# yesint/molar

Measured on AMD Instinct MI355X. Metric: frames/sec + Matom-pairs/sec, 1M-atom PBC neighbor search + RMSD fit, higher is better.
Workload: dtype f32; 1 GPU; 1M-atom synthetic triclinic box A, per frame: PBC neighbour search rc=1.2 nm (ordered pair list in HBM) + Kabsch RMSD fit/COM/gyration of a 100k-atom selection; natoms=1000000, selection_atoms=100000, frames_per_gpu=1451, parallelism=frames sharded over 1 rank(s), no data-path collective, streams_per_gpu=2, measure_overlapped_with_search=True

## Files before the change

molar_amd/csrc/pair_kernels.hpp:

```cpp
#pragma once

#include "boxmath.hpp"
#include "common.hpp"

namespace mh {
namespace pairk {

enum { MODE_COUNT = 0, MODE_FILL = 1, MODE_HIST = 2 };

#ifndef MH_COUNT_WPE
#define MH_COUNT_WPE 6
#endif
#ifndef MH_FILL_WPE
#define MH_FILL_WPE 8
#endif
#ifndef MH_WPB
#define MH_WPB 1
#endif
constexpr int waves_per_block(int mode) { return mode == MODE_HIST ? 4 : MH_WPB; }
constexpr int KREG = 8;
constexpr int FIFO_CAP = 128;
#ifndef MOLAR_HIP_NO_WIDE_FLUSH
#define MOLAR_HIP_WIDE_FLUSH 1
#endif
constexpr int FIFO_WIDE = 256;
constexpr uint32_t XCD_RUN = 128;
constexpr float F32_EPS = 1.1920929e-07f;
constexpr bool MASKED_COUNT_SORTED = true;

static __constant__ uint8_t MASKS[14][6] = {
    {0, 0, 0, 0, 0, 0},
    {0, 0, 0, 1, 0, 0}, {0, 0, 0, 0, 1, 0}, {0, 0, 0, 0, 0, 1},
    {0, 0, 0, 1, 1, 0}, {0, 0, 0, 1, 0, 1}, {0, 0, 0, 0, 1, 1},
    {0, 0, 0, 1, 1, 1},
    {1, 0, 0, 0, 1, 0}, {1, 0, 0, 0, 0, 1}, {0, 1, 0, 0, 0, 1},
    {1, 1, 0, 0, 0, 1}, {1, 0, 1, 0, 1, 0}, {0, 1, 1, 1, 0, 0},
};


typedef float v4f_t __attribute__((ext_vector_type(4)));
__device__ __forceinline__ float4 gload4(const float4 *p, size_t i) {
    const v4f_t v = ((const __attribute__((address_space(1))) v4f_t *)p)[i];
    return make_float4(v.x, v.y, v.z, v.w);
}
__device__ __forceinline__ uint32_t gload_u32(const uint32_t *p, size_t i) {
    return ((const __attribute__((address_space(1))) uint32_t *)p)[i];
}
__device__ __forceinline__ void gstore_u32(uint32_t *p, size_t i, uint32_t v) {
    ((__attribute__((address_space(1))) uint32_t *)p)[i] = v;
}
__device__ __forceinline__ float uniform_f32(float v) { return __uint_as_float(__builtin_amdgcn_readfirstlane(__float_as_uint(v))); }
__device__ __forceinline__ float4 lload4(const float4 *p, uint32_t i) {
    const v4f_t v = ((const __attribute__((address_space(3))) v4f_t *)p)[i];
    return make_float4(v.x, v.y, v.z, v.w);
}

struct SearchParams {
    const float4 *sa;
    const float4 *sb;
    const uint32_t *csa;
    const uint32_t *csb;
    const float *vdwa;
    const float *vdwb;
    const float4 *aabb_b;
    const float4 *perm_b;
    const float4 *chunk_aabb_b;
    const uint4 *h16_b;
    const float4 *cell_org_b;
    uint32_t mfma_count;
    const struct TaskDesc *task_desc;
    uint32_t *maskbuf;
    const unsigned long long *task_moff;
    unsigned long long mask_cap_units;
    unsigned long long out_cap;
    uint32_t dx, dy, dz;
    uint32_t pbc;
    uint32_t use_box;
    uint32_t nblocks;
    uint32_t wrap_kind;
    uint32_t prune_wrapped;
    float prune_limit2;
    uint32_t approx_wrapped;
    float band_lo, band_hi;
    uint32_t hist_nbins;
    float hist_min, hist_max;
    unsigned long long *hist_bins;
    unsigned long long *hist_total;
    const float *hist_edges;
    float hist_scale;
    uint32_t hist_lean;
    const uint32_t *hist_nslots;
#ifdef MOLAR_HIP_DEBUG_KNOBS
    uint32_t debug_skip;
    unsigned long long *dbg;
#endif
    float cutoff2;
    uint64_t ntasks;
    molar_hip_box box;
    alignas(16) float shifts4[96];
    uint32_t hist_big;
};

struct TaskDesc {
    uint32_t a0, n1, b0, n2, cb, flags, pad0, pad1;
};

struct SlotDesc {
    uint32_t a0, n1, b0, n2;
    uint32_t cb, flags, i0, frame;
    unsigned long long moff, pad1;
};
static_assert(sizeof(SlotDesc) == 48, "SlotDesc is read with three 16-byte loads");

struct Task {
    uint32_t a0, n1, b0, n2;
    uint32_t rps;
    uint32_t cb;
    uint32_t ca;
    uint32_t wrap_b;
    uint32_t wrap;
    bool tri;
    bool valid;
};

template <int KIND, bool UNIFORM>
__device__ __forceinline__ Task decode_task(const SearchParams &P, uint64_t t) {
    Task T;
    T.valid = false;
    T.tri = false;
    T.a0 = T.b0 = T.n1 = T.n2 = 0;
    T.cb = 0;
    T.ca = 0;
    T.wrap_b = 0;
    T.rps = 64u;
    T.wrap = 0;
    uint32_t half = 0;
    uint64_t e = t;
    if (KIND != MOLAR_HIP_SEARCH_SINGLE) {
        half = (uint32_t)(t & 1ull);
        e = t >> 1;
    }
    const uint32_t m = (uint32_t)(e % 14ull);
    const uint64_t cidx = e / 14ull;
    const uint32_t z = (uint32_t)(cidx % P.dz);
    const uint64_t r = cidx / P.dz;
    const uint32_t y = (uint32_t)(r % P.dy);
    const uint32_t x = (uint32_t)(r / P.dy);
    const uint32_t dims[3] = {P.dx, P.dy, P.dz};
    uint32_t c[2][3] = {{x + MASKS[m][0], y + MASKS[m][1], z + MASKS[m][2]},
                        {x + MASKS[m][3], y + MASKS[m][4], z + MASKS[m][5]}};
    uint32_t wrap = 0, wrap_c2 = 0;
    for (int i = 0; i < 2; ++i)
        for (int d = 0; d < 3; ++d)
            if (c[i][d] == dims[d]) {
                if ((P.pbc >> d) & 1u) {
                    c[i][d] = 0;
                    wrap |= 1u << d;
                    if (i == 1) wrap_c2 |= 1u << d;
                } else {
                    return T;
                }
            }
    const uint32_t i1 = c[0][0] + c[0][1] * P.dx + c[0][2] * P.dx * P.dy;
    const uint32_t i2 = c[1][0] + c[1][1] * P.dx + c[1][2] * P.dx * P.dy;
    uint32_t ca = i1, cb = i2;
    if (KIND == MOLAR_HIP_SEARCH_SINGLE) {
        T.tri = (i1 == i2);
    } else if (half) {
        ca = i2;
        cb = i1;
    }
    T.a0 = P.csa[ca];
    T.n1 = P.csa[ca + 1] - T.a0;
    T.b0 = P.csb[cb];
    T.n2 = P.csb[cb + 1] - T.b0;
    T.wrap = wrap;
    T.wrap_b = (KIND != MOLAR_HIP_SEARCH_SINGLE && half) ? (wrap & ~wrap_c2) : wrap_c2;
    T.rps = (P.use_box && wrap == MOLAR_HIP_PBC_FULL && P.box.nshift != 0 && T.n1 <= 4096u) ? (T.n1 <= 1024u ? 2u : 8u) : 64u;
    T.cb = cb;
    T.ca = ca;
    if (UNIFORM) {
        T.cb = __builtin_amdgcn_readfirstlane(T.cb);
        T.rps = __builtin_amdgcn_readfirstlane(T.rps);
        T.a0 = __builtin_amdgcn_readfirstlane(T.a0);
        T.n1 = __builtin_amdgcn_readfirstlane(T.n1);
        T.b0 = __builtin_amdgcn_readfirstlane(T.b0);
        T.n2 = __builtin_amdgcn_readfirstlane(T.n2);
        T.wrap = __builtin_amdgcn_readfirstlane(T.wrap);
    }
    T.valid = T.n1 > 0 && T.n2 > 0 && !(T.tri && T.n1 < 2);
    return T;
}

typedef float v2f __attribute__((ext_vector_type(2)));

enum { WK_NONE = 0, WK_DIAG = 1, WK_UPPER = 2, WK_GENERAL = 3 };

__device__ __forceinline__ v2f round_away2(v2f f) { return v2f{__builtin_roundf(f.x), __builtin_roundf(f.y)}; }

struct BoxRegs {
    float I[9], M[9];
    int nshift;
};

template <int WK, bool WIDE4 = false>
__device__ __forceinline__ v2f pair_d2x2(const SearchParams &P, const BoxRegs &B, uint32_t wrap, float px, float py,
                                         float pz, v2f qx, v2f qy, v2f qz) {
// ... 602 lines not shown
    typedef __attribute__((address_space(3))) uint32_t lds_u32;
    typedef __attribute__((address_space(1))) u4_t glb_u4;
    const float cutoff2 = P.cutoff2;
    const uint32_t rows = __builtin_amdgcn_readfirstlane(T.n1 - i0 < 64u ? T.n1 - i0 : 64u);
    const uint32_t kh = lane >> 5, cl = lane & 31u;
    const uint32_t nct = (T.n2 + 31u) >> 5, nch = (T.n2 + 63u) >> 6;
    float Sx = 0.f, Sy = 0.f, Sz = 0.f;
    for (int d = 0; d < 3; ++d) {
        if (!((T.wrap >> d) & 1u)) continue;
        const float sgn = ((T.wrap_b >> d) & 1u) ? 1.0f : -1.0f;
        Sx += sgn * P.box.m[3 * d];
        Sy += sgn * P.box.m[3 * d + 1];
        Sz += sgn * P.box.m[3 * d + 2];
    }
    float4 a = make_float4(0.f, 0.f, 0.f, 0.f);
    if (lane < rows) a = gload4(P.sa, T.a0 + i0 + lane);
    const float4 org = gload4(P.cell_org_b, T.cb);
    const float4 blo = gload4(P.aabb_b, 2 * T.cb), bhi = gload4(P.aabb_b, 2 * T.cb + 1);
    const bool need = lane < rows && !(aabb_d2(a.x - Sx, a.y - Sy, a.z - Sz, blo.x, blo.y, blo.z, bhi.x, bhi.y, bhi.z) > P.prune_limit2);
    const unsigned long long live = __builtin_amdgcn_ballot_w64(need);
    const uint32_t nlive = (uint32_t)__popcll(live);
    if (nlive == 0u) {
        count_out = 0u;
        return true;
    }
    const uint32_t rank = __builtin_amdgcn_mbcnt_hi((uint32_t)(live >> 32), __builtin_amdgcn_mbcnt_lo((uint32_t)live, 0u));
    const float r0 = (a.x - Sx) - org.x, r1 = (a.y - Sy) - org.y, r2 = (a.z - Sz) - org.z;
    float ra2 = need ? (r0 * r0 + r1 * r1) + r2 * r2 : 0.0f;
    float big = need ? fmaxf(fmaxf(fabsf(a.x), fabsf(a.y)), fabsf(a.z)) : 0.0f;
    const bool fin = ra2 == ra2;
    for (int off = 32; off > 0; off >>= 1) {
        ra2 = fmaxf(ra2, __shfl_xor(ra2, off, 64));
        big = fmaxf(big, __shfl_xor(big, off, 64));
    }
    const float R = 1.0001f * __builtin_sqrtf(ra2) + org.w;
    const float rc = __builtin_sqrtf(P.band_hi);
    const float L = (fmaxf(fmaxf(fabsf(org.x), fabsf(org.y)), fabsf(org.z)) + R) + (fmaxf(fmaxf(fabsf(Sx), fabsf(Sy)), fabsf(Sz)) + big);
    const float Em = mfma_error_bound(R, cutoff2);
    const float E = uniform_f32((P.band_hi - cutoff2) * 1.0001f + Em + 4.0f * (5.9604645e-08f * (2.0f * L + 2.0f * rc)) * rc);
    if (__builtin_amdgcn_ballot_w64(!fin || !(E == E) || !mfma_bound_usable(R, Em, cutoff2) || !(E < 0.06f * cutoff2)) != 0ull) return false;
    u4_t bq[MFMA_TILES];
#pragma unroll
    for (int t = 0; t < MFMA_TILES; ++t) {
        const uint32_t col = (uint32_t)t * 32u + cl;
        if (32u * (uint32_t)(t + 1) <= T.n2) {
            bq[t] = ((const glb_u4 *)P.h16_b)[T.b0 + col];
        } else {
            bq[t] = u4_t{0u, 0u, 0u, 0x00007BFFu};
            if (col < T.n2) bq[t] = ((const glb_u4 *)P.h16_b)[T.b0 + col];
        }
    }
    {
        ((lds_u4 *)lh)[2u * lane] = u4_t{0u, 0u, 0u, 0x00007BFFu};
        ((lds_u4 *)lh)[2u * lane + 1u] = u4_t{0u, 0u, 0u, 0x3C003C00u};
        __builtin_amdgcn_wave_barrier();
        if (need) {
            const _Float16 h0 = (_Float16)r0, h1 = (_Float16)r1, h2 = (_Float16)r2;
            const _Float16 l0 = (_Float16)(r0 - (float)h0), l1 = (_Float16)(r1 - (float)h1), l2 = (_Float16)(r2 - (float)h2);
            const float e0 = (float)h0 + (float)l0, e1 = (float)h1 + (float)l1, e2 = (float)h2 + (float)l2;
            const float na = ((e0 * e0 + e1 * e1) + e2 * e2) - cutoff2;
            const _Float16 nh = (_Float16)na, nl = (_Float16)(na - (float)nh);
            const _Float16 m2 = (_Float16)-2.0f;
            const _Float16 g0 = m2 * h0, g1 = m2 * h1, g2 = m2 * h2, s0 = m2 * l0, s1 = m2 * l1, s2 = m2 * l2;
            ((lds_u4 *)lh)[2u * rank] = u4_t{pack_h2(g0, g1), pack_h2(g2, g0), pack_h2(g1, g2), pack_h2(nh, nl)};
            ((lds_u4 *)lh)[2u * rank + 1u] = u4_t{pack_h2(s0, s1), pack_h2(s2, s0), pack_h2(s1, s2), 0x3C003C00u};
            la[rank] = a;
        }
    }
    __builtin_amdgcn_wave_barrier();
    const u4_t a0q = ((const lds_u4 *)lh)[2u * cl + kh], a1q = ((const lds_u4 *)lh)[2u * (32u + cl) + kh];
    const v8h_t A0 = __builtin_bit_cast(v8h_t, a0q), A1 = __builtin_bit_cast(v8h_t, a1q);
    __builtin_amdgcn_wave_barrier();
    lds_u32 *todo = (lds_u32 *)lh;
    constexpr uint32_t TODO_CAP = 512u;
    uint32_t ntodo = 0, cnt = 0;
    const uint32_t ngroups = nlive > 32u ? 2u : 1u;
    auto block = [&](int t, int rt) __attribute__((always_inline)) -> uint32_t {
        u4_t bt = bq[t];
        if (kh == 0u) bt.w = 0x3C003C00u;
        const v16f_t zero = {0.f, 0.f, 0.f, 0.f, 0.f, 0.f, 0.f, 0.f, 0.f, 0.f, 0.f, 0.f, 0.f, 0.f, 0.f, 0.f};
        const v16f_t acc = __builtin_amdgcn_mfma_f32_32x32x16_f16(rt == 0 ? A0 : A1, __builtin_bit_cast(v8h_t, bt), zero, 0, 0, 0);
        uint32_t h = 0u;
        float m = INFINITY;
#pragma unroll
        for (int i = 0; i < 16; ++i) {
            h = __builtin_amdgcn_alignbit(h, __float_as_uint(acc[i]), 31);
            m = __builtin_fminf(m, __builtin_fabsf(acc[i]));
        }
        if (__builtin_amdgcn_ballot_w64(m < E) != 0ull) {
            uint32_t bm = 0u;
#pragma unroll
            for (int i = 0; i < 16; ++i) {
                const bool ib = __builtin_fabsf(acc[i]) < E;
                bm = (bm << 1) | (ib ? 1u : 0u);
                const unsigned long long mk = __builtin_amdgcn_ballot_w64(ib);
                if (mk) {
                    const uint32_t at = ntodo + __builtin_amdgcn_mbcnt_hi((uint32_t)(mk >> 32), __builtin_amdgcn_mbcnt_lo((uint32_t)mk, 0u));
                    const uint32_t rl = 32u * (uint32_t)rt + 8u * (uint32_t)(i / 4) + 4u * kh + (uint32_t)(i % 4);
                    if (ib && at < TODO_CAP) todo[at] = (rl << 16) | (32u * (uint32_t)t + cl);
                    ntodo += (uint32_t)__popcll(mk);
                }
            }
            h &= ~bm;
        }
        return h;
    };
    auto spread = [](uint32_t x) -> uint32_t {
        x = (x | (x << 8)) & 0x00FF00FFu;
        return (x | (x << 4)) & 0x0F0F0F0Fu;
    };
#pragma unroll
    for (int k = 0; k < MFMA_TILES / 2; ++k) {
        if ((uint32_t)k < nch) {
#pragma unroll
            for (int rt = 0; rt < 2; ++rt) {
                if ((uint32_t)rt >= ngroups) continue;
                const uint32_t hx = block(2 * k, rt);
                const uint32_t hy = (uint32_t)(2 * k + 1) < nct ? block(2 * k + 1, rt) : 0u;
                const uint32_t got = (uint32_t)__shfl_xor((int)(kh ? hx : hy), 32, 64);
                const uint32_t half0 = kh ? got : hx, half1 = kh ? hy : got;
                const uint32_t word = (spread(half0) << 4) | spread(half1);
                cnt += (uint32_t)__popc(word);
                gstore_u32(mwords, ((uint32_t)rt * nch + (uint32_t)k) * 64u + lane, word);
            }
        }
    }
    if (ntodo > TODO_CAP) return false;
    if (ntodo) {
        asm volatile("s_waitcnt vmcnt(0)" ::: "memory");
        __builtin_amdgcn_wave_barrier();
        for (uint32_t q0 = 0; q0 < ntodo; q0 += 64u) {
            bool hx = false;
            uint32_t rl = 0u, col = 0u;
            if (q0 + lane < ntodo) {
                const uint32_t e = todo[q0 + lane];
                rl = e >> 16;
                col = e & 0xFFFFu;
                if (rl < nlive && col < T.n2) {
                    const float4 b = gload4(P.sb, T.b0 + col);
                    const float4 p = lload4(la, rl);
                    hx = wrapped_d2_exact(P, T.wrap, b.x - p.x, b.y - p.y, b.z - p.z) <= cutoff2;
                }
            }
            if (hx) atomicOr(mwords + ((rl >> 5) * nch + (col >> 6)) * 64u + (col & 63u), 0x80000000u >> (rl & 31u));
            const unsigned long long mx = __builtin_amdgcn_ballot_w64(hx);
            if (lane == 0) cnt += (uint32_t)__popcll(mx);
        }
    }
    for (int off = 32; off > 0; off >>= 1) cnt += __shfl_xor(cnt, off, 64);
    count_out = cnt;
    return true;
}

template <int KIND, bool FILL, bool WRAPPED, int NCH, bool TRI, bool MASKED>
__device__ __forceinline__ uint32_t run_fast(const SearchParams &P, const Task &T, uint32_t i0, Fifo &F, float4 *la,
                                             uint32_t lane, uint32_t *mwords) {
    static_assert(!(WRAPPED && TRI), "a triangular (same-cell) entry never wraps on the fast path");
    if constexpr (!FILL && !WRAPPED && MASKED_COUNT_SORTED) return run_count_sorted<KIND, NCH, TRI>(P, T, i0, la, lane);
    const bool approx = WRAPPED && P.approx_wrapped != 0u && !(P.box.nshift != 0 && T.wrap == MOLAR_HIP_PBC_FULL);
    float Sx = 0.f, Sy = 0.f, Sz = 0.f;
    if (WRAPPED && approx) {
        for (int d = 0; d < 3; ++d) {
            if (!((T.wrap >> d) & 1u)) continue;
            const float sgn = ((T.wrap_b >> d) & 1u) ? 1.0f : -1.0f;
            Sx += sgn * P.box.m[3 * d];
            Sy += sgn * P.box.m[3 * d + 1];
            Sz += sgn * P.box.m[3 * d + 2];
        }
    }
    constexpr bool REPLAY = FILL && MASKED;
    float bx[NCH], by[NCH], bz[NCH];
    uint32_t bid[NCH];
    if (!REPLAY) {
#pragma unroll
        for (int k = 0; k < NCH; ++k) {
            const uint32_t jj = (uint32_t)k * 64u + lane;
            float4 q = make_float4(3.0e38f, 3.0e38f, 3.0e38f, 0.f);
            if (jj < T.n2) {
                q = gload4(P.sb, T.b0 + jj);
                if (WRAPPED) { q.x += Sx; q.y += Sy; q.z += Sz; }
            }
            bx[k] = q.x; by[k] = q.y; bz[k] = q.z; bid[k] = __float_as_uint(q.w);
        }
    }
    const float cutoff2 = P.cutoff2;
    const float band_lo = P.band_lo, band_hi = P.band_hi;
    const uint32_t rows = __builtin_amdgcn_readfirstlane(T.n1 - i0 < T.rps ? T.n1 - i0 : T.rps);
    unsigned long long live;
    {
        float4 a = make_float4(0.f, 0.f, 0.f, 0.f);
        if (lane < rows) a = gload4(P.sa, T.a0 + i0 + lane);
        la[lane] = a;
        const float4 lo = gload4(P.aabb_b, 2 * T.cb), hi = gload4(P.aabb_b, 2 * T.cb + 1);
        bool need = true;
        if (TRI) {
        } else if (!WRAPPED) {
            need = !(aabb_d2(a.x, a.y, a.z, lo.x, lo.y, lo.z, hi.x, hi.y, hi.z) > cutoff2);
        } else if (approx) {
            need = !(aabb_d2(a.x - Sx, a.y - Sy, a.z - Sz, lo.x, lo.y, lo.z, hi.x, hi.y, hi.z) > P.prune_limit2);
        }
        live = __builtin_amdgcn_ballot_w64(lane < rows && need);
    }
    __builtin_amdgcn_wave_barrier();
    uint32_t total = 0;

    if (REPLAY) {
        if (!mwords) return 0u;
        F.recompute = WRAPPED ? 1u : 2u;
        F.la = la;
        F.wrap = T.wrap;
        F.fq = F.fq_store;
        float4 q[NCH];
#pragma unroll
        for (int k = 0; k < NCH; ++k) {
            const uint32_t jj = (uint32_t)k * 64u + lane;
            q[k] = make_float4(0.f, 0.f, 0.f, 0.f);
            if (jj < T.n2) q[k] = gload4(P.sb, T.b0 + jj);
        }
        uint32_t w[NCH];
        uint32_t nrow = 0;
        while (live) {
            if ((nrow & 31u) == 0u) {
#pragma unroll
                for (int k = 0; k < NCH; ++k) w[k] = gload_u32(mwords, ((nrow >> 5) * NCH + k) * 64u + lane);
            }
            ++nrow;
            const uint32_t r = (uint32_t)__builtin_ctzll(live);
            live &= ~(1ull << r);
#pragma unroll
            for (int k = 0; k < NCH; ++k) {
                const bool hit = (int32_t)w[k] < 0;
                w[k] += w[k];
                const unsigned long long mask = __builtin_amdgcn_ballot_w64(hit);
                if (mask) {
                    const uint32_t cnt = (uint32_t)__popcll(mask);
                    if (hit) {
                        const uint32_t s = __builtin_amdgcn_mbcnt_hi((uint32_t)(mask >> 32),
                                                                     __builtin_amdgcn_mbcnt_lo((uint32_t)mask, F.tail)) &
                                           (FIFO_CAP - 1);
                        F.fq[s] = q[k];
                        F.fd[s] = r;
                    }
                    F.tail += cnt;
                    total += cnt;
                    if (F.tail - F.head >= 64u) fifo_drain<KIND>(P, F, lane);
                }
            }
        }
        if (F.tail != F.head) {
            __builtin_amdgcn_wave_barrier();
            fifo_flush<KIND>(P, F, F.tail - F.head, lane);
        }
        F.recompute = 0u;
        F.fq = nullptr;
        return total;
    }

#ifdef MOLAR_HIP_WIDE_FLUSH
    constexpr bool WIDE = FILL && !WRAPPED && KIND != MOLAR_HIP_SEARCH_WITHIN;
#else
    constexpr bool WIDE = false;
#endif
    if (FILL) {
        F.recompute = (WRAPPED && approx) ? 1u : 0u;
        F.la = la;
        F.wrap = T.wrap;
        if (WIDE && !F.hist) F.quota = 128u - ((uint32_t)F.base & 127u);
    }
    uint32_t acc = 0;
    uint32_t acc_hi = 0;
    uint32_t hw[NCH];
    uint32_t su = 0, mu = 0;
    uint32_t nrow = 0;
    if (MASKED) {
#pragma unroll
        for (int k = 0; k < NCH; ++k) hw[k] = 0u;
    }
    auto store_group = [&](uint32_t g, uint32_t n) {
#pragma unroll
        for (int k = 0; k < NCH; ++k) {
            acc += (uint32_t)__popc(hw[k]);
            if (mwords) gstore_u32(mwords, (g * NCH + k) * 64u + lane, hw[k] << (32u - n));
            hw[k] = 0u;
        }
    };
    auto exact_d2 = [&](const float4 &p, uint32_t jj) -> float {
        float4 q = make_float4(3.0e38f, 3.0e38f, 3.0e38f, 0.f);
        if (jj < T.n2) q = gload4(P.sb, T.b0 + jj);
        return wrapped_d2_exact(P, T.wrap, q.x - p.x, q.y - p.y, q.z - p.z);
    };
    while (live) {
        const uint32_t r = (uint32_t)__builtin_ctzll(live);
        live &= ~(1ull << r);
        const float4 p = lload4(la, r);
        const uint32_t id_i = __float_as_uint(p.w);
        const uint32_t i = i0 + r;
#pragma unroll
        for (int k = 0; k < NCH; ++k) {
            if (TRI && (uint32_t)k * 64u + 63u <= i) {
                if (MASKED && !FILL) hw[k] += hw[k];
                continue;
            }
            const uint32_t jj = (uint32_t)k * 64u + lane;
            const float dx = bx[k] - p.x, dy = by[k] - p.y, dz = bz[k] - p.z;
            float d2 = (dx * dx + dy * dy) + dz * dz;
            if (WRAPPED && !approx) d2 = wrapped_d2_exact<FILL && !MASKED>(P, T.wrap, dx, dy, dz);
            if (TRI && (uint32_t)k * 64u <= i) d2 = (jj > i) ? d2 : INFINITY;
            if (!FILL) {
                if (MASKED) {
                    if (WRAPPED && approx) {
                        unsigned long long scr;
                        asm volatile("v_cmp_gt_f32 vcc, %4, %3\n\t"
                                     "v_addc_co_u32 %0, %2, %0, %0, vcc\n\t"
                                     "v_addc_co_u32 %1, %2, %1, %1, vcc"
                                     : "+v"(hw[k]), "+v"(su), "=&s"(scr) : "v"(d2), "s"(band_lo) : "vcc");
                        asm volatile("v_cmp_ge_f32 vcc, %2, %1\n\tv_addc_co_u32 %0, vcc, %0, %0, vcc" : "+v"(mu) : "v"(d2), "s"(band_hi) : "vcc");
                    } else {
                        asm volatile("v_cmp_ge_f32 vcc, %2, %1\n\tv_addc_co_u32 %0, vcc, %0, %0, vcc" : "+v"(hw[k]) : "v"(d2), "s"(cutoff2) : "vcc");
                    }
                } else if (WRAPPED && approx) {
                    asm volatile("v_cmp_gt_f32 vcc, %2, %1\n\tv_addc_co_u32 %0, vcc, 0, %0, vcc" : "+v"(acc) : "v"(d2), "s"(band_lo) : "vcc");
                    asm volatile("v_cmp_ge_f32 vcc, %2, %1\n\tv_addc_co_u32 %0, vcc, 0, %0, vcc" : "+v"(acc_hi) : "v"(d2), "s"(band_hi) : "vcc");
                } else {
                    asm volatile("v_cmp_ge_f32 vcc, %2, %1\n\tv_addc_co_u32 %0, vcc, 0, %0, vcc" : "+v"(acc) : "v"(d2), "s"(cutoff2) : "vcc");
                }
            } else {
                bool hit;
                uint32_t third = __float_as_uint(d2);
                if (WRAPPED && approx) {
                    const bool sure = d2 < band_lo, maybe = d2 <= band_hi;
                    hit = sure;
                    if (__builtin_amdgcn_ballot_w64(maybe && !sure)) hit = sure || (maybe && exact_d2(p, jj) <= cutoff2);
                    third = (r << 26) | (T.b0 + jj);
                } else {
                    hit = d2 <= cutoff2;
                }
                const unsigned long long mask = __builtin_amdgcn_ballot_w64(hit);
                if (mask) {
                    const uint32_t cnt = (uint32_t)__popcll(mask);
                    if (hit) {
                        const uint32_t rank = __builtin_amdgcn_mbcnt_hi((uint32_t)(mask >> 32), __builtin_amdgcn_mbcnt_lo((uint32_t)mask, 0u));
                        const uint32_t off = ((rank + F.tail) << 2) & (((WIDE ? FIFO_WIDE : FIFO_CAP) - 1u) << 2);
                        typedef __attribute__((address_space(3))) uint32_t lds_u32;
                        *(lds_u32 *)((__attribute__((address_space(3))) char *)F.fi + off) = id_i;
                        *(lds_u32 *)((__attribute__((address_space(3))) char *)F.fj + off) = bid[k];
                        *(lds_u32 *)((__attribute__((address_space(3))) char *)F.fd + off) = third;
                    }
                    F.tail += cnt;
                    total += cnt;
                    if (WIDE) {
                        if (F.tail - F.head >= 128u) fifo_drain_wide<KIND>(P, F, lane);
                    } else if (F.tail - F.head >= 64u) fifo_drain<KIND>(P, F, lane);
                }
            }
        }
        if (!FILL && WRAPPED && approx) {
            bool any_amb;
            if (MASKED) {
                any_amb = __builtin_amdgcn_ballot_w64(((su ^ mu) & ((1u << NCH) - 1u)) != 0u) != 0ull;
            } else {
                any_amb = __builtin_amdgcn_ballot_w64(acc != acc_hi) != 0ull;
            }
            if (any_amb) {
#pragma unroll
                for (int k = 0; k < NCH; ++k) {
                    const float dx = bx[k] - p.x, dy = by[k] - p.y, dz = bz[k] - p.z;
                    const float d2 = (dx * dx + dy * dy) + dz * dz;
                    const bool amb = d2 <= band_hi && !(d2 < band_lo);
                    if (__builtin_amdgcn_ballot_w64(amb)) {
                        if (amb && exact_d2(p, (uint32_t)k * 64u + lane) <= cutoff2) {
                            if (MASKED) hw[k] |= 1u;
                            else acc += 1u;
                        }
                    }
                }
                acc_hi = acc;
            }
        }
        if (!FILL && MASKED) {
            if ((++nrow & 31u) == 0u) store_group((nrow >> 5) - 1u, 32u);
        }
    }
    if (!FILL) {
        if (MASKED && (nrow & 31u) != 0u) store_group(nrow >> 5, nrow & 31u);
        for (int off = 32; off > 0; off >>= 1) acc += __shfl_xor(acc, off, 64);
        total = acc;
    } else if (F.tail != F.head) {
        __builtin_amdgcn_wave_barrier();
        if (WIDE) {
            while (F.tail != F.head) {
                const uint32_t c = F.tail - F.head < 64u ? F.tail - F.head : 64u;
                fifo_flush<KIND, FIFO_WIDE>(P, F, c, lane);
            }
        } else {
            fifo_flush<KIND>(P, F, F.tail - F.head, lane);
        }
    }
    if (FILL) F.recompute = 0u;
    return total;
}

constexpr int KMAX_WIDE = 16;
constexpr int KMAX_HUGE = 32;
template <int KIND, bool FILL, int WK, bool MASKED, int KMAX = KREG>
__device__ __forceinline__ uint32_t run_task_nch(const SearchParams &P, const Task &T, uint32_t i0, Fifo &F, float4 *la,
                                                 uint32_t lane, uint32_t *mwords) {
    const uint32_t nchunks = (T.n2 + 63u) >> 6;
    if constexpr (KMAX > KMAX_WIDE) {
        if ((KIND == MOLAR_HIP_SEARCH_SINGLE || KIND == MOLAR_HIP_SEARCH_DOUBLE) && nchunks > (uint32_t)KREG && nchunks <= (uint32_t)KMAX) {
            constexpr bool WR = WK != WK_NONE;
            const bool tri = KIND == MOLAR_HIP_SEARCH_SINGLE && WK == WK_NONE && T.tri;
            if (!T.tri || tri) {
#define MH_HUGE_CASE(N)                                                                                              \
    if (nchunks <= (uint32_t)(N)) {                                                                                  \
        if (tri) {                                                                                                   \
            if constexpr (KIND == MOLAR_HIP_SEARCH_SINGLE && WK == WK_NONE)                                          \
                return run_fast<KIND, FILL, false, N, true, false>(P, T, i0, F, la, lane, nullptr);                  \
        }                                                                                                            \
        return run_fast<KIND, FILL, WR, N, false, false>(P, T, i0, F, la, lane, nullptr);                            \
    }
                MH_HUGE_CASE(16) MH_HUGE_CASE(20) MH_HUGE_CASE(24) MH_HUGE_CASE(28) MH_HUGE_CASE(32)
#undef MH_HUGE_CASE
            }
        }
    } else if constexpr (KMAX > KREG) {
        if ((KIND == MOLAR_HIP_SEARCH_SINGLE || KIND == MOLAR_HIP_SEARCH_DOUBLE) && nchunks > (uint32_t)KREG && nchunks <= (uint32_t)KMAX) {
            constexpr bool WR = WK != WK_NONE;
            const bool tri = KIND == MOLAR_HIP_SEARCH_SINGLE && WK == WK_NONE && T.tri;
            if (!T.tri || tri) {
#define MH_WIDE_CASE(N)                                                                                              \
    case N:                                                                                                          \
        if (tri) {                                                                                                   \
            if constexpr (KIND == MOLAR_HIP_SEARCH_SINGLE && WK == WK_NONE)                                          \
                return run_fast<KIND, FILL, false, N, true, false>(P, T, i0, F, la, lane, nullptr);                  \
        }                                                                                                            \
        return run_fast<KIND, FILL, WR, N, false, false>(P, T, i0, F, la, lane, nullptr);
                switch (nchunks) {
                    MH_WIDE_CASE(9) MH_WIDE_CASE(10) MH_WIDE_CASE(11) MH_WIDE_CASE(12)
                    MH_WIDE_CASE(13) MH_WIDE_CASE(14) MH_WIDE_CASE(15)
                    default: break;
                }
                if (tri) {
                    if constexpr (KIND == MOLAR_HIP_SEARCH_SINGLE && WK == WK_NONE)
                        return run_fast<KIND, FILL, false, 16, true, false>(P, T, i0, F, la, lane, nullptr);
                }
                return run_fast<KIND, FILL, WR, 16, false, false>(P, T, i0, F, la, lane, nullptr);
#undef MH_WIDE_CASE
            }
        }
    }
    if constexpr (!FILL && WK == WK_NONE && (KIND == MOLAR_HIP_SEARCH_SINGLE || KIND == MOLAR_HIP_SEARCH_DOUBLE)) {
        if ((P.mfma_count & 1u) && F.lh && T.n2 <= 32u * (uint32_t)MFMA_TILES) {
            bool done = true;
            const uint32_t cm = (KIND == MOLAR_HIP_SEARCH_SINGLE && T.tri) ? run_count_mfma<KIND, true>(P, T, i0, la, F.lh, lane, done)
                                                                          : run_count_mfma<KIND, false>(P, T, i0, la, F.lh, lane, done);
            if (done) return cm;
        }
    }
    if constexpr (!FILL && MASKED && WK != WK_NONE && (KIND == MOLAR_HIP_SEARCH_SINGLE || KIND == MOLAR_HIP_SEARCH_DOUBLE)) {
        if ((P.mfma_count & 2u) && F.lh && mwords && !T.tri && T.rps == 64u && T.n2 <= 32u * (uint32_t)MFMA_TILES && P.approx_wrapped != 0u &&
            !(P.box.nshift != 0 && T.wrap == MOLAR_HIP_PBC_FULL)) {
            uint32_t cw = 0u;
            if (run_count_mfma_wrapped<KIND>(P, T, i0, la, F.lh, lane, mwords, cw)) return cw;
            __builtin_amdgcn_wave_barrier();
        }
    }
    if ((KIND == MOLAR_HIP_SEARCH_SINGLE || KIND == MOLAR_HIP_SEARCH_DOUBLE) && !T.tri && nchunks <= (uint32_t)KREG) {
        constexpr bool WR = WK != WK_NONE;
        switch (nchunks) {
            case 1: return run_fast<KIND, FILL, WR, 1, false, MASKED && WR>(P, T, i0, F, la, lane, mwords);
            case 2: return run_fast<KIND, FILL, WR, 2, false, MASKED && WR>(P, T, i0, F, la, lane, mwords);
            case 3: return run_fast<KIND, FILL, WR, 3, false, MASKED && WR>(P, T, i0, F, la, lane, mwords);
            case 4: return run_fast<KIND, FILL, WR, 4, false, MASKED && WR>(P, T, i0, F, la, lane, mwords);
            case 5: return run_fast<KIND, FILL, WR, 5, false, MASKED && WR>(P, T, i0, F, la, lane, mwords);
            case 6: return run_fast<KIND, FILL, WR, 6, false, MASKED && WR>(P, T, i0, F, la, lane, mwords);
            case 7: return run_fast<KIND, FILL, WR, 7, false, MASKED && WR>(P, T, i0, F, la, lane, mwords);
            default: return run_fast<KIND, FILL, WR, 8, false, MASKED && WR>(P, T, i0, F, la, lane, mwords);
        }
    }
    if (KIND == MOLAR_HIP_SEARCH_SINGLE && WK == WK_NONE && T.tri && nchunks <= (uint32_t)KREG) {
        switch (nchunks) {
            case 1: return run_fast<KIND, FILL, false, 1, true, false>(P, T, i0, F, la, lane, mwords);
            case 2: return run_fast<KIND, FILL, false, 2, true, false>(P, T, i0, F, la, lane, mwords);
            case 3: return run_fast<KIND, FILL, false, 3, true, false>(P, T, i0, F, la, lane, mwords);
            case 4: return run_fast<KIND, FILL, false, 4, true, false>(P, T, i0, F, la, lane, mwords);
            case 5: return run_fast<KIND, FILL, false, 5, true, false>(P, T, i0, F, la, lane, mwords);
            case 6: return run_fast<KIND, FILL, false, 6, true, false>(P, T, i0, F, la, lane, mwords);
            case 7: return run_fast<KIND, FILL, false, 7, true, false>(P, T, i0, F, la, lane, mwords);
            default: return run_fast<KIND, FILL, false, 8, true, false>(P, T, i0, F, la, lane, mwords);
        }
    }
    if (nchunks > (uint32_t)KREG) {
        if (KIND == MOLAR_HIP_SEARCH_SINGLE && T.tri) return run_task<KIND, FILL, WK, true, 0, false, FILL && !MASKED>(P, T, i0, F, lane);
        return run_task<KIND, FILL, WK, false, 0, false, FILL && !MASKED>(P, T, i0, F, lane);
    }
    if (KIND == MOLAR_HIP_SEARCH_SINGLE && T.tri) return run_task<KIND, FILL, WK, true, KREG, true, FILL && !MASKED>(P, T, i0, F, lane);
    return run_task<KIND, FILL, WK, false, KREG, true, FILL && !MASKED>(P, T, i0, F, lane);
}

template <int KIND>
__global__ void __launch_bounds__(256) plan_kernel(SearchParams P, uint32_t *__restrict__ task_nb,
                                                   TaskDesc *__restrict__ task_desc, uint32_t *__restrict__ task_mu,
                                                   uint32_t fast_kind, uint32_t *__restrict__ slot_cnt, uint64_t nslot_cnt,
                                                   unsigned long long *__restrict__ scan_state, uint64_t nstate,
                                                   SearchParams *__restrict__ params_dst) {
    const uint64_t t = (uint64_t)blockIdx.x * blockDim.x + threadIdx.x;
    if (t < nslot_cnt) slot_cnt[t] = 0u;
    if (t < nstate) scan_state[t] = 0ull;
    if (params_dst && blockIdx.x == 0) {
        const uint32_t *src = (const uint32_t *)__builtin_amdgcn_kernarg_segment_ptr();
        uint32_t *d = (uint32_t *)params_dst;
        for (uint32_t w = threadIdx.x; w < (uint32_t)(sizeof(SearchParams) / 4u); w += blockDim.x) d[w] = src[w];
    }
    if (t == P.ntasks) {
        task_nb[t] = 0u;
        task_mu[t] = 0u;
    }
    if (t >= P.ntasks) return;
    const Task T = decode_task<KIND, false>(P, t);
    const uint32_t nb = T.valid ? (T.n1 + T.rps - 1u) / T.rps : 0u;
    task_nb[t] = nb;
    const uint32_t nch = (T.n2 + 63u) >> 6;
    task_mu[t] = (fast_kind && P.use_box && T.wrap != 0u && nch <= (uint32_t)KREG) ? nb * 2u * nch : 0u;
    TaskDesc d;
    d.a0 = T.a0; d.n1 = T.n1; d.b0 = T.b0; d.n2 = T.n2; d.cb = T.cb;
    d.flags = T.wrap | (T.tri ? 0x100u : 0u) | (T.valid ? 0x200u : 0u) | (T.wrap_b << 12) | (T.rps << 16);
    d.pad0 = d.pad1 = 0;
    task_desc[t] = d;
}

static __global__ void __launch_bounds__(256) slotmap_kernel(uint64_t ntasks, const uint32_t *__restrict__ task_first,
                                                      const TaskDesc *__restrict__ task_desc,
                                                      const unsigned long long *__restrict__ task_moff,
                                                      SlotDesc *__restrict__ slot_desc, uint64_t nslots_bound,
                                                      unsigned long long *__restrict__ sizes_host) {
    const uint64_t t = (uint64_t)blockIdx.x * blockDim.x + threadIdx.x;
    if (t == 0 && sizes_host) {
        sizes_host[1] = task_moff ? task_moff[ntasks] : 0ull;
        sizes_host[2] = task_first[ntasks];
    }
    if (t >= ntasks) {
        const uint64_t s = (uint64_t)task_first[ntasks] + (t - ntasks);
        if (s <= nslots_bound) {
            SlotDesc z;
            z.a0 = z.n1 = z.b0 = z.n2 = z.cb = z.flags = z.i0 = z.frame = 0u;
            z.moff = ~0ull >> 1;
            z.pad1 = 0ull;
            slot_desc[s] = z;
        }
        return;
    }
    const uint32_t s0 = task_first[t], s1 = task_first[t + 1];
    if (s1 == s0) return;
    const TaskDesc d = task_desc[t];
    const uint32_t rps = d.flags >> 16, nch = (d.n2 + 63u) >> 6;
    const unsigned long long m0 = task_moff ? task_moff[t] : (~0ull >> 1);
    for (uint32_t s = s0; s < s1; ++s) {
        SlotDesc o;
        o.a0 = d.a0; o.n1 = d.n1; o.b0 = d.b0; o.n2 = d.n2;
        o.cb = d.cb; o.flags = d.flags; o.i0 = (s - s0) * rps; o.frame = 0u;
        o.moff = task_moff ? m0 + (unsigned long long)(s - s0) * 2u * nch : m0;
        o.pad1 = 0ull;
        slot_desc[s] = o;
    }
}

template <int KIND>
__device__ __forceinline__ bool hist_lean_slot(const SearchParams &P, uint32_t flags, uint32_t n2) {
    if (KIND != MOLAR_HIP_SEARCH_SINGLE && KIND != MOLAR_HIP_SEARCH_DOUBLE) return false;
    if (((n2 + 63u) >> 6) > (uint32_t)KREG && !P.hist_big) return false;
    const uint32_t wrap = flags & 7u;
    if (!(P.use_box && wrap != 0u)) return true;
    if (flags & 0x100u) return false;
    return P.approx_wrapped != 0u && !(P.box.nshift != 0 && wrap == MOLAR_HIP_PBC_FULL);
}

template <int KIND, int MODE, int WPE = 0>
__global__ void __launch_bounds__(64 * waves_per_block(MODE))
__attribute__((amdgpu_waves_per_eu(WPE ? WPE : (MODE == MODE_HIST ? 4 : (MODE == MODE_COUNT ? MH_COUNT_WPE : MH_FILL_WPE))))) pair_kernel(const SearchParams *__restrict__ Pp,
                                                     const SlotDesc *__restrict__ slot_desc,
                                                     const uint32_t nslots_arg,
                                                     uint32_t *__restrict__ slot_cnt,
                                                     const unsigned long long *__restrict__ slot_base,
                                                     uint2 *__restrict__ out_pairs, float *__restrict__ out_dist,
                                                     uint32_t *__restrict__ out_ids) {
    constexpr int WAVES_PER_BLOCK = waves_per_block(MODE), BLOCK = 64 * WAVES_PER_BLOCK;
    constexpr int PLANE = MODE != MODE_COUNT ? FIFO_WIDE : FIFO_CAP;
    static_assert(FIFO_CAP * 16 <= 2 * FIFO_WIDE * 4, "the replay queue fits in two planes");
    __shared__ __attribute__((aligned(16))) uint32_t lds[WAVES_PER_BLOCK][3][PLANE];
    __shared__ float4 lds_a[WAVES_PER_BLOCK][64];
    __shared__ uint4 lds_h[MODE == MODE_COUNT ? WAVES_PER_BLOCK : 1][MODE == MODE_COUNT ? 128 : 1];
    constexpr bool FILL = MODE != MODE_COUNT;
    extern __shared__ uint32_t lds_hist[];
    const SearchParams &P0 = *Pp;
#ifdef MH_SLOT_LOOP
    uint32_t lane_var = threadIdx.x & 63u;
    const uint32_t &lane = lane_var;
#else
    const uint32_t lane = threadIdx.x & 63u;
#endif
    uint32_t nslots = nslots_arg;
    if (MODE == MODE_HIST && P0.hist_nslots) {
        const uint32_t real = __builtin_amdgcn_readfirstlane(P0.hist_nslots[0]);
        nslots = real < nslots_arg ? real : nslots_arg;
    }
    const uint32_t wave = WAVES_PER_BLOCK == 1 ? 0u : __builtin_amdgcn_readfirstlane(threadIdx.x >> 6);
    constexpr bool hist = MODE == MODE_HIST;
    if (hist) {
        for (uint32_t b = threadIdx.x; b < P0.hist_nbins; b += BLOCK) lds_hist[b] = 0u;
        __syncthreads();
    }
    unsigned long long wave_total = 0;
    auto process_slot = [&](uint32_t w) __attribute__((always_inline)) {
        uint32_t wr = w;
        {
            const uint32_t x = w & 7u, q = w >> 3;
            const uint32_t full = (nslots / (8u * XCD_RUN)) * (8u * XCD_RUN);
            if (w < full) wr = ((q / XCD_RUN) * 8u + x) * XCD_RUN + (q % XCD_RUN);
        }
// ... 158 lines not shown
```

Measured before the change: 756.7 frames/s.

## Compact B-cell columns against the live-row bounding box in the fill pass

In the fill pass for plain non-wrapped, non-triangular entries, a wave-wide AABB of the live A rows is reduced with DPP min/max. Each B atom is then tested against that box, and only the surviving B atoms are compacted through an LDS ring buffer into fewer 64-wide register chunks before the pair loop. This is meant to cut distance tests and fill iterations on B atoms that cannot be within the cutoff. The cost is an extra sweep over B, an extra load of B, inline-asm DPP reductions, ballot-based compaction and more template instantiations.

```diff
diff --git a/molar_amd/csrc/pair_kernels.hpp b/molar_amd/csrc/pair_kernels.hpp
--- a/molar_amd/csrc/pair_kernels.hpp
+++ b/molar_amd/csrc/pair_kernels.hpp
@@ -16,6 +16,9 @@
 #endif
 #ifndef MH_WPB
 #define MH_WPB 1
+#endif
+#ifndef MH_FILL_COLUMNS
+#define MH_FILL_COLUMNS 1
 #endif
 constexpr int waves_per_block(int mode) { return mode == MODE_HIST ? 4 : MH_WPB; }
 constexpr int KREG = 8;
@@ -53,6 +56,9 @@
 __device__ __forceinline__ float4 lload4(const float4 *p, uint32_t i) {
     const v4f_t v = ((const __attribute__((address_space(3))) v4f_t *)p)[i];
     return make_float4(v.x, v.y, v.z, v.w);
+}
+__device__ __forceinline__ void lstore4(float4 *p, uint32_t i, const float4 &q) {
+    ((__attribute__((address_space(3))) v4f_t *)p)[i] = v4f_t{q.x, q.y, q.z, q.w};
 }
 
 struct SearchParams {
@@ -961,10 +967,119 @@
     return true;
 }
 
-template <int KIND, bool FILL, bool WRAPPED, int NCH, bool TRI, bool MASKED>
+struct Columns {
+    unsigned long long live;
+    uint32_t keep;
+    uint32_t nsrc;
+};
+
+__device__ __forceinline__ void wave_box(float &lx, float &ly, float &lz, float &hx, float &hy, float &hz) {
+#define MH_BOX_STEP(CTRL)                                      \
+    asm volatile("s_nop 1\n\t"                                 \
+                 "v_min_f32_dpp %0, %0, %0 " CTRL "\n\t"       \
+                 "v_min_f32_dpp %1, %1, %1 " CTRL "\n\t"       \
+                 "v_min_f32_dpp %2, %2, %2 " CTRL "\n\t"       \
+                 "v_max_f32_dpp %3, %3, %3 " CTRL "\n\t"       \
+                 "v_max_f32_dpp %4, %4, %4 " CTRL "\n\t"       \
+                 "v_max_f32_dpp %5, %5, %5 " CTRL                \
+                 : "+v"(lx), "+v"(ly), "+v"(lz), "+v"(hx), "+v"(hy), "+v"(hz));
+    MH_BOX_STEP("quad_perm:[1,0,3,2] row_mask:0xf bank_mask:0xf")
+    MH_BOX_STEP("quad_perm:[2,3,0,1] row_mask:0xf bank_mask:0xf")
+    MH_BOX_STEP("row_half_mirror row_mask:0xf bank_mask:0xf")
+    MH_BOX_STEP("row_mirror row_mask:0xf bank_mask:0xf")
+    MH_BOX_STEP("row_bcast:15 row_mask:0xa bank_mask:0xf")
+    MH_BOX_STEP("row_bcast:31 row_mask:0xc bank_mask:0xf")
+#undef MH_BOX_STEP
+    auto last = [](float v) { return __int_as_float(__builtin_amdgcn_readlane(__float_as_int(v), 63)); };
+    lx = last(lx); ly = last(ly); lz = last(lz); hx = last(hx); hy = last(hy); hz = last(hz);
+}
+
+template <int KIND>
+__device__ __forceinline__ uint32_t column_sweep(const SearchParams &P, const Task &T, uint32_t i0, float4 *la, uint32_t lane,
+                                                 Columns &C) {
+    const float cutoff2 = P.cutoff2;
+    const uint32_t rows = __builtin_amdgcn_readfirstlane(T.n1 - i0 < T.rps ? T.n1 - i0 : T.rps);
+    float4 a = make_float4(0.f, 0.f, 0.f, 0.f);
+    if (lane < rows) a = gload4(P.sa, T.a0 + i0 + lane);
+    la[lane] = a;
+    const float4 lo = gload4(P.aabb_b, 2 * T.cb), hi = gload4(P.aabb_b, 2 * T.cb + 1);
+    float4 q[KREG];
+#pragma unroll
+    for (int k = 0; k < KREG; ++k) {
+        const uint32_t jj = (uint32_t)k * 64u + lane;
+        q[k] = make_float4(3.0e38f, 3.0e38f, 3.0e38f, 0.f);
+        if (jj < T.n2) q[k] = gload4(P.sb, T.b0 + jj);
+    }
+    const bool need = lane < rows && !(aabb_d2(a.x, a.y, a.z, lo.x, lo.y, lo.z, hi.x, hi.y, hi.z) > cutoff2);
+    C.live = __builtin_amdgcn_ballot_w64(need);
+    C.nsrc = (T.n2 + 63u) >> 6;
+    C.keep = 0u;
+    if (C.live == 0ull) return 0u;
+    float lx = need ? a.x : INFINITY, ly = need ? a.y : INFINITY, lz = need ? a.z : INFINITY;
+    float hx = need ? a.x : -INFINITY, hy = need ? a.y : -INFINITY, hz = need ? a.z : -INFINITY;
+    wave_box(lx, ly, lz, hx, hy, hz);
+    uint32_t kept = 0u;
+#pragma unroll
+    for (int k = 0; k < KREG; ++k) {
+        if ((uint32_t)k < C.nsrc) {
+            const bool kp = (uint32_t)k * 64u + lane < T.n2 && !(aabb_d2(q[k].x, q[k].y, q[k].z, lx, ly, lz, hx, hy, hz) > cutoff2);
+            kept += (uint32_t)__popcll(__builtin_amdgcn_ballot_w64(kp));
+            C.keep |= kp ? (1u << k) : 0u;
+        }
+    }
+    return kept;
+}
+
+template <int NCH>
+__device__ __forceinline__ void load_columns(const SearchParams &P, const Task &T, const Columns &C, float4 *ring, uint32_t lane,
+                                             float (&bx)[NCH], float (&by)[NCH], float (&bz)[NCH], uint32_t (&bid)[NCH]) {
+    const float4 *mine = P.sb + T.b0 + lane;
+    const uint32_t n2 = T.n2;
+    auto fetch = [&](uint32_t s) -> float4 {
+        float4 q = make_float4(3.0e38f, 3.0e38f, 3.0e38f, 0.f);
+        if (s * 64u + lane < n2) q = gload4(mine, s * 64u);
+        return q;
+    };
+    if (C.nsrc == (uint32_t)NCH) {
+#pragma unroll
+        for (int k = 0; k < NCH; ++k) {
+            const float4 q = fetch((uint32_t)k);
+            bx[k] = q.x; by[k] = q.y; bz[k] = q.z; bid[k] = __float_as_uint(q.w);
+        }
+        return;
+    }
+    uint32_t src = 0u, head = 0u, tail = 0u;
+    float4 qn = fetch(0u);
+#pragma unroll
+    for (int kk = 0; kk < NCH; ++kk) {
+        while (tail - head < 64u && src < C.nsrc) {
+            const float4 qs = qn;
+            const bool kp = ((C.keep >> src) & 1u) != 0u;
+            ++src;
+            if (src < C.nsrc) qn = fetch(src);
+            const unsigned long long mask = __builtin_amdgcn_ballot_w64(kp);
+            if (mask) {
+                if (kp) {
+                    const uint32_t rank = __builtin_amdgcn_mbcnt_hi((uint32_t)(mask >> 32), __builtin_amdgcn_mbcnt_lo((uint32_t)mask, 0u));
+                    lstore4(ring, (tail + rank) & 127u, qs);
+                }
+                tail += (uint32_t)__popcll(mask);
+            }
+        }
+        __builtin_amdgcn_wave_barrier();
+        float4 v = make_float4(3.0e38f, 3.0e38f, 3.0e38f, 0.f);
+        if (head + lane < tail) v = lload4(ring, (head + lane) & 127u);
+        head = tail - head < 64u ? tail : head + 64u;
+        __builtin_amdgcn_wave_barrier();
+        bx[kk] = v.x; by[kk] = v.y; bz[kk] = v.z; bid[kk] = __float_as_uint(v.w);
+    }
+}
+
+template <int KIND, bool FILL, bool WRAPPED, int NCH, bool TRI, bool MASKED, bool COLS = false>
 __device__ __forceinline__ uint32_t run_fast(const SearchParams &P, const Task &T, uint32_t i0, Fifo &F, float4 *la,
-                                             uint32_t lane, uint32_t *mwords) {
+                                             uint32_t lane, uint32_t *mwords, const Columns *cols = nullptr) {
     static_assert(!(WRAPPED && TRI), "a triangular (same-cell) entry never wraps on the fast path");
+    static_assert(!COLS || (FILL && !WRAPPED && !TRI && !MASKED), "column compaction: plain entries of the fill pass");
     if constexpr (!FILL && !WRAPPED && MASKED_COUNT_SORTED) return run_count_sorted<KIND, NCH, TRI>(P, T, i0, la, lane);
     const bool approx = WRAPPED && P.approx_wrapped != 0u && !(P.box.nshift != 0 && T.wrap == MOLAR_HIP_PBC_FULL);
     float Sx = 0.f, Sy = 0.f, Sz = 0.f;
@@ -980,7 +1095,9 @@
     constexpr bool REPLAY = FILL && MASKED;
     float bx[NCH], by[NCH], bz[NCH];
     uint32_t bid[NCH];
-    if (!REPLAY) {
+    if constexpr (COLS) {
+        load_columns<NCH>(P, T, *cols, F.fq_store, lane, bx, by, bz, bid);
+    } else if (!REPLAY) {
 #pragma unroll
         for (int k = 0; k < NCH; ++k) {
             const uint32_t jj = (uint32_t)k * 64u + lane;
@@ -996,7 +1113,9 @@
     const float band_lo = P.band_lo, band_hi = P.band_hi;
     const uint32_t rows = __builtin_amdgcn_readfirstlane(T.n1 - i0 < T.rps ? T.n1 - i0 : T.rps);
     unsigned long long live;
-    {
+    if constexpr (COLS) {
+        live = cols->live;
+    } else {
         float4 a = make_float4(0.f, 0.f, 0.f, 0.f);
         if (lane < rows) a = gload4(P.sa, T.a0 + i0 + lane);
         la[lane] = a;
@@ -1274,6 +1393,25 @@
             __builtin_amdgcn_wave_barrier();
         }
     }
+#if MH_FILL_COLUMNS
+    if constexpr (FILL && MASKED && WK == WK_NONE && KMAX == KREG && (KIND == MOLAR_HIP_SEARCH_SINGLE || KIND == MOLAR_HIP_SEARCH_DOUBLE)) {
+        if (!T.tri && nchunks > 1u && nchunks <= (uint32_t)KREG) {
+            Columns C;
+            const uint32_t kept = column_sweep<KIND>(P, T, i0, la, lane, C);
+            if (kept == 0u) return 0u;
+            switch ((kept + 63u) >> 6) {
+                case 1: return run_fast<KIND, true, false, 1, false, false, true>(P, T, i0, F, la, lane, nullptr, &C);
+                case 2: return run_fast<KIND, true, false, 2, false, false, true>(P, T, i0, F, la, lane, nullptr, &C);
+                case 3: return run_fast<KIND, true, false, 3, false, false, true>(P, T, i0, F, la, lane, nullptr, &C);
+                case 4: return run_fast<KIND, true, false, 4, false, false, true>(P, T, i0, F, la, lane, nullptr, &C);
+                case 5: return run_fast<KIND, true, false, 5, false, false, true>(P, T, i0, F, la, lane, nullptr, &C);
+                case 6: return run_fast<KIND, true, false, 6, false, false, true>(P, T, i0, F, la, lane, nullptr, &C);
+                case 7: return run_fast<KIND, true, false, 7, false, false, true>(P, T, i0, F, la, lane, nullptr, &C);
+                default: return run_fast<KIND, true, false, 8, false, false, true>(P, T, i0, F, la, lane, nullptr, &C);
+            }
+        }
+    }
+#endif
     if ((KIND == MOLAR_HIP_SEARCH_SINGLE || KIND == MOLAR_HIP_SEARCH_DOUBLE) && !T.tri && nchunks <= (uint32_t)KREG) {
         constexpr bool WR = WK != WK_NONE;
         switch (nchunks) {
```

Result: no change. 758.6 frames/s (median of 4 runs) (+0.2%).
